# Enigmatisms/AdaPT

Hardware: AMD Instinct MI355X
Metric: Msamples/s (W*H*spp/s), unidirectional MIS path tracing (higher is better)
Workload: dtype f32

## Files before the change

adapt_amd/_lib.py:

```python
from __future__ import annotations

import ctypes as C
import os

_HERE = os.path.dirname(os.path.abspath(__file__))
LIB_PATHS = {"fast": os.environ.get("ADAPT_MI_LIB") or os.path.join(_HERE, "libadapt_mi.so"),
             "exact": os.environ.get("ADAPT_MI_LIB_EXACT") or os.path.join(_HERE, "libadapt_mi_exact.so")}
_variant = "exact" if os.environ.get("APT_EXACT", "0") not in ("", "0") else "fast"
LIB_PATH = LIB_PATHS[_variant]

f32p = C.POINTER(C.c_float)
i32p = C.POINTER(C.c_int32)
u32p = C.POINTER(C.c_uint32)
u8p = C.POINTER(C.c_uint8)
f64p = C.POINTER(C.c_double)
APT_N_KERNELS = 5
KERNEL_NAMES = ("generate", "extend", "shade", "shadow", "finalize")


class AptError(RuntimeError):
    pass


class SceneDesc(C.Structure):
# ... 78 lines not shown
    "apt_device_ptr": (C.c_int, [C.c_void_p, C.POINTER(C.c_void_p), i32p]),
    "apt_stream": (C.c_int, [C.c_void_p, C.POINTER(C.c_void_p)]),
    "apt_intersect": (C.c_int, [C.c_void_p, C.c_int32, f32p, f32p, i32p, f32p, f32p]),
    "apt_occluded": (C.c_int, [C.c_void_p, C.c_int32, f32p, f32p, f32p, i32p]),
    "apt_rng_stream": (C.c_int, [C.c_int32, C.c_uint32, C.c_uint32, C.c_uint32, C.c_int32, u32p]),
    "apt_bxdf_probe": (C.c_int, [C.c_int32, C.c_int32, i32p, f32p, f32p, C.c_float, C.c_int32, C.c_uint32, f32p]),
    "apt_medium_probe": (C.c_int, [C.c_int32, C.c_int32, i32p, f32p, C.c_int32, f32p, C.c_uint32, f32p]),
    "apt_volume_probe": (C.c_int, [C.c_int32, C.c_int32, i32p, f32p, f32p, C.c_int32, f32p, C.c_uint32, f32p]),
    "apt_emitter_probe": (C.c_int, [C.c_void_p, C.c_int32, f32p, C.c_uint32, f32p]),
    "apt_texture_probe": (C.c_int, [C.c_void_p, C.c_int32, i32p, f32p, f32p]),
    "apt_surface_maps_probe": (C.c_int, [C.c_void_p, C.c_int32, i32p, f32p, f32p]),
    "apt_transient_bin_probe": (C.c_int, [C.c_int32, C.c_int32, f32p, C.c_float, C.c_float, C.c_int32, i32p]),
    "apt_renderer_info": (C.c_int, [C.c_void_p, i32p, i32p, C.POINTER(C.c_int64), i32p, C.POINTER(C.c_char_p), i32p]),
    "apt_renderer_camera_fused": (C.c_int, [C.c_void_p, i32p]),
    "apt_renderer_record_staged": (C.c_int, [C.c_void_p, i32p]),
    "apt_measure_sclk_mhz": (C.c_int, [C.c_int32, f32p]),
    "apt_last_error": (C.c_char_p, []),
    "apt_version": (C.c_char_p, []),
}

_libs = {}


def use(variant: str) -> str:
    global _variant, LIB_PATH
    if variant not in LIB_PATHS:
        raise ValueError(f"unknown build variant {variant!r}")
    prev, _variant = _variant, variant
    LIB_PATH = LIB_PATHS[variant]
    return prev
# ... 36 lines not shown
```

adapt_amd/csrc/api.hip:

```cpp
#include <hip/hip_runtime.h>
#include <chrono>

#include <algorithm>
#include <cmath>
#include <cstdio>
#include <cstdlib>
#include <cstring>
#include <limits>
#include <memory>
#include <string>
#include <vector>

#include "../../include/adapt_mi.h"
#include "bvh_build.hpp"
#include "shade_stage.hpp"
#include "unit_kernels.hpp"
#include "aov.hpp"
#include "volumetric.hpp"

#define APT_EXPORT extern "C" __attribute__((visibility("default")))

static thread_local std::string g_err;
static int fail(int code, const std::string& msg) { g_err = msg; return code; }
#define HIP_TRY(expr)                                                                              \
// ... 166 lines not shown
enum Pipeline { PIPE_STAGED, PIPE_SORTED, PIPE_TRACED, PIPE_VOLUMETRIC };

struct apt_renderer {
    const apt_scene* scene = nullptr;
    apt_render_cfg cfg{};
    Params par{};
    int n_cols = 0, npix = 0, spp_batch = 1;
    int cnt = 0;
    std::vector<Lane> lanes;
    int n_lanes = 1;
    hipStream_t stream() const { return lanes[0].stream; }
    DevBuf accum, scratch, pix_key;
    DevBuf cam_strips;
    int record_stage = 0;
    shade_traced_fn traced_fn = nullptr;
    int camera_fuse = 0;
    Counters host_counters{};
    int grid_small = 0, grid_trace = 0, nq = APT_MAX_NQ;
    const ShadeVariant* shade = nullptr;
    int trace_mode = TRACE_BVH;
    int trace_nt = BLOCK;
    int trace_items = BLOCK;
    Pipeline pipeline = PIPE_STAGED;
    int dyn_fetch = 0;
    bool tile_ok = false;
    extend_fn extend = nullptr, fix = nullptr;
    int ovf_levels = 0;
    int n_cq = 0;
    int vev_single = 0;
    vev_shade_fn vev_all = nullptr;
// ... 578 lines not shown
    cf.inv_focal = c.inv_focal; cf.half_w = c.half_w; cf.half_h = c.half_h;
    cf.width = c.width; cf.height = c.height; cf.n_cols = owned_columns(c); cf.band_width = c.band_width; cf.rank = c.rank; cf.world = c.world_size;
    return cf;
}
static int make_camera_strips(apt_renderer* r) {
    if (r->pipeline != PIPE_TRACED) return APT_OK;
    const apt_scene* sc = r->scene;
    const bool cull = !(getenv("APT_CAMERA_CULL") && atoi(getenv("APT_CAMERA_CULL")) == 0);
    std::vector<uint64_t> masks;
    if (apt::camera_strips(sc->h_prims.data(), sc->n_prims, sc->h_flat_recs, sc->h_flat_tab, sc->h_flat_counts, cam_film(r->cfg), cull, masks) != 0)
        return fail(APT_E_INVALID, "apt_renderer_create: camera strip lists: bad record or film");
    hipError_t e = upload(r->cam_strips, masks);
    if (e != hipSuccess) return fail(APT_E_HIP, std::string("upload camera strip lists: ") + hipGetErrorString(e));
    const bool want = !(getenv("APT_CAMERA_FUSE") && atoi(getenv("APT_CAMERA_FUSE")) == 0);
    r->camera_fuse = (want && !r->adaptive && !r->par.do_crop && r->par.max_bounce >= 1 && r->shade->traced_cam != nullptr) ? 1 : 0;
    return APT_OK;
}

APT_EXPORT int apt_camera_strips(const float* prims, int32_t n_prims, const int32_t* obj_info, int32_t n_objects, const apt_render_cfg* cfg, int32_t cull,
                                 uint64_t* masks, int32_t masks_cap, int32_t* n_strips, int32_t* n_pairs) {
    if (!prims || !obj_info || !cfg || n_prims <= 0 || n_objects <= 0 || !n_strips || !n_pairs) return fail(APT_E_INVALID, "apt_camera_strips: bad argument");
    apt_render_cfg c = *cfg;
    if (c.world_size <= 0) { c.world_size = 1; c.rank = 0; }
    if (c.band_width <= 0) c.band_width = c.width;
    if (c.width <= 0 || c.height <= 0 || c.rank < 0 || c.rank >= c.world_size || owned_columns(c) <= 0) return fail(APT_E_INVALID, "apt_camera_strips: bad film or rank");
    std::vector<float> st, tb; int cn[7];
    if (apt::build_flat(prims, n_prims, obj_info, n_objects, nullptr, st, tb, cn) != 0) return fail(APT_E_INVALID, "apt_camera_strips: obj_info range outside the primitive array");
    std::vector<uint64_t> m;
    if (apt::camera_strips(prims, n_prims, st, tb, cn, cam_film(c), cull != 0, m) != 0) return fail(APT_E_INVALID, "apt_camera_strips: bad record or film");
    *n_strips = (int32_t)m.size();
// ... 409 lines not shown
    int done = 0, batch = 0;
    hipEvent_t prev_fin = nullptr;
    const int batch_cap = lane_batch(r, n_spp);
    while (done < n_spp) {
        const int B = (n_spp - done < batch_cap) ? (n_spp - done) : batch_cap;
        Lane& ln = r->lanes[(size_t)(batch % r->n_lanes)];
        hipStream_t st = ln.stream;
        const Queues& q = ln.q;
        Counters* cnt = ln.cnt();
        Params p = r->par; p.cnt_base = r->cnt; p.spp_batch = B;
        const size_t total = (size_t)r->npix * (size_t)B;
        if (int rc = begin_batch(r, ln)) return rc;
#if APT_FAST
        if (r->pipeline == PIPE_TRACED) {
            const unsigned long long* strips = r->cam_strips.as<unsigned long long>();
            int cur = 0, b0 = 0;
            if (r->camera_fuse) {
                { LaunchTimer t(r, APT_K_SHADE, st); hipLaunchKernelGGL(r->shade->traced_cam, dim3(grid_for(total, r->grid_small, nq)), dim3(BLOCK), 0, st, sc, p, q, cnt, strips); }
                { LaunchTimer t(r, APT_K_SHADE, st); hipLaunchKernelGGL(r->traced_fn, dim3(r->grid_fix), dim3(BLOCK), 0, st, sc, p, q, cnt, 0, 0); }
                cur = 1; b0 = 1;
            } else {
                LaunchTimer t(r, APT_K_GENERATE, st);
                if (r->adaptive) hipLaunchKernelGGL(k_generate_trace_ad, dim3(grid_for(total, r->grid_small, 1)), dim3(BLOCK), 0, st, sc, p, q, cnt, (const uint8_t*)r->aq.active, strips);
                else hipLaunchKernelGGL(k_generate_trace, dim3(grid_for(total, r->grid_small, 1)), dim3(BLOCK), 0, st, sc, p, q, cnt, strips);
            }
            for (int b = b0; b < p.max_bounce; b++) {
                { LaunchTimer t(r, APT_K_SHADE, st); hipLaunchKernelGGL(r->traced_fn, dim3(grid_for(total, r->grid_small, nq)), dim3(BLOCK), 0, st, sc, p, q, cnt, cur, b); }
                cur ^= 1;
            }
            if (p.max_bounce > 0) { LaunchTimer t(r, APT_K_SHADOW, st, false); hipLaunchKernelGGL(r->fix, dim3(r->grid_fix), dim3(BLOCK), 0, st, sc, p, q, cnt, cur, (const uint32_t*)cnt->n_active[cur], ln.plan); }
// ... 533 lines not shown
    }
    std::vector<unsigned long long> h((size_t)n_waves * 2);
    HIP_TRY(hipMemcpy(h.data(), out.p, h.size() * 8, hipMemcpyDeviceToHost));
    std::vector<double> r;
    for (int w = 0; w < n_waves; w++) if (h[2 * (size_t)w + 1] > 0) r.push_back(100.0 * (double)h[2 * (size_t)w] / (double)h[2 * (size_t)w + 1]);
    if (r.empty()) return fail(APT_E_STATE, "apt_measure_sclk_mhz: the wall clock did not advance");
    std::nth_element(r.begin(), r.begin() + r.size() / 2, r.end());
    *mhz = (float)r[r.size() / 2];
    return APT_OK;
}
APT_EXPORT int apt_renderer_camera_fused(const apt_renderer* r, int32_t* out) {
    if (!r || !out) return fail(APT_E_INVALID, "apt_renderer_camera_fused: null argument");
    *out = r->camera_fuse;
    return APT_OK;
}
APT_EXPORT int apt_renderer_record_staged(const apt_renderer* r, int32_t* out) {
    if (!r || !out) return fail(APT_E_INVALID, "apt_renderer_record_staged: null argument");
    *out = r->record_stage;
    return APT_OK;
}
APT_EXPORT int apt_renderer_info(const apt_renderer* r, int32_t* spp_batch, int32_t* n_subqueues, int64_t* queue_bytes, int32_t* lds_bytes, const char** shade_variant, int32_t* trace_mode) {
    if (!r) return fail(APT_E_INVALID, "apt_renderer_info: null handle");
    if (spp_batch) *spp_batch = r->spp_batch;
    if (n_subqueues) *n_subqueues = r->nq;
    if (queue_bytes) *queue_bytes = (int64_t)r->lanes[0].pool.bytes * (int64_t)r->lanes.size();
    if (lds_bytes) *lds_bytes = (int32_t)r->lds_bytes;
    if (shade_variant) *shade_variant = r->shade_name.c_str();
    if (trace_mode) *trace_mode = r->trace_mode;
    return APT_OK;
}
// ... 1 lines not shown
```

adapt_amd/csrc/shade_stage.hpp:

```cpp
#pragma once
#include "stages.hpp"

APT_D float ti_fmod(float a, float b) { float q = floorf(a / b); return a - b * q; }
APT_D f3 mix3(f3 a, f3 b, float t) { return a * (1.0f - t) + b * t; }
APT_D f3 texture_query(const DevScene& sc, int map, int obj, float u, float v) {
    const int* ti_ = sc.tex_i + 15 * obj + 5 * map; const float* tf = sc.tex_f + 6 * obj + 2 * map;
    const float w = (float)ti_[3], h = (float)ti_[4];
    const float scaled_u = ti_fmod((u * tf[0]) * w, w - 1.f), scaled_v = ti_fmod((v * tf[1]) * h, h - 1.f);
    float floor_u = floorf(scaled_u), floor_v = floorf(scaled_v);
    const float ratio_u = fmaxf(scaled_u - floor_u, 0.f), ratio_v = fmaxf(scaled_v - floor_v, 0.f);
    floor_u = fminf(fmaxf(floor_u, 0.f), w - 1.f); floor_v = fminf(fmaxf(floor_v, 0.f), h - 1.f);
    const float ceil_u = fminf(floor_u + 1.f, w - 1.f), ceil_v = fminf(floor_v + 1.f, h - 1.f);
    const int fu = (int)(floor_u + (float)ti_[1]), fv = (int)(floor_v + (float)ti_[2]), cu = (int)(ceil_u + (float)ti_[1]), cv = (int)(ceil_v + (float)ti_[2]);
    const float* img = sc.atlas[map]; const int W = sc.atlas_w[map];
    const float* r0 = img + (size_t)fv * W * 3; const float* r1 = img + (size_t)cv * W * 3;
    const f3 q_ff = ld3(r0 + 3 * fu), q_cf = ld3(r0 + 3 * cu), q_fc = ld3(r1 + 3 * fu), q_cc = ld3(r1 + 3 * cu);
    return mix3(mix3(q_ff, q_cf, ratio_u), mix3(q_fc, q_cc, ratio_u), ratio_v);
}
APT_D bool get_uv_item(const DevScene& sc, int map, int obj, int prim, float bu, float bv, f3& out) {
    if (sc.atlas[map] == nullptr || !(sc.tex_i[15 * obj + 5 * map] > -255)) return false;
    const float* uv = sc.uvs + 6 * prim;
    const float w0 = 1.f - bu - bv;
    const float gu = (uv[2] * bu + uv[4] * bv) + uv[0] * w0, gv = (uv[3] * bu + uv[5] * bv) + uv[1] * w0;
    out = texture_query(sc, map, obj, gu, gv);
// ... 50 lines not shown
    if (old >= epoch) {
        while (__hip_atomic_load(&cnt->fix_done[sq * CNT_PAD], __ATOMIC_ACQUIRE, __HIP_MEMORY_SCOPE_AGENT) < epoch) __builtin_amdgcn_s_sleep(16);
        return;
    }
    const uint32_t qbase = (uint32_t)sq * p.subcap, sh_qbase = (uint32_t)sq * q.sh_subcap;
    const bool need_uv = sc.has_vn || sc.tex_i != nullptr;
    for (uint32_t base = 0; base < n_def; base += 64u) {
        const uint32_t li = base + lane_id(); const bool valid = li < n_def;
        const uint32_t lj = valid ? li : n_def - 1u;
        const uint32_t io = (q.tr_stage_top ? qbase + p.subcap - n_def + lj : (uint32_t)ncls * p.cap + qbase + lj) << 4;
        const float4 ra = ldq(q.tr[cur][0], io), rb = ldq(q.tr[cur][1], io), rc = ldq(q.tr[cur][2], io), rd = ldq(q.tr[cur][3], io);
        const f3 o = mk3(ra.x, ra.y, ra.z), d = mk3(rb.x, rb.y, rb.z);
        HitRec r0, r1; r0.t = r1.t = 1e7f; r0.prim = r1.prim = -1; r0.u = r0.v = r1.u = r1.v = 0.f;
        int c0, c1;
        flat_closest2(sc.flat, sc.sweep, sc.prim_class, o, d, o, d, r0, r1, c0, c1);
        if (valid && r0.prim >= 0) {
            const int oc = ncls > 1 ? c0 : 0;
            const uint32_t pos = atomicAdd(&cnt->n_tr[bounce % 3][oc][sq * CNT_PAD], 1u);
            const uint32_t slot = (uint32_t)oc * p.cap + qbase + pos, so = slot << 4;
            stq(q.tr[cur][0], so, make_float4(ra.x, ra.y, ra.z, r0.t));
            stq(q.tr[cur][1], so, make_float4(rb.x, rb.y, rb.z, __uint_as_float((__float_as_uint(rb.w) & ~0xffu) | (uint32_t)r0.prim)));
            stq(q.tr[cur][2], so, rc); stq(q.tr[cur][3], so, rd);
            if (need_uv) { float2 uv_; uv_.x = r0.u; uv_.y = r0.v; stq(q.tr_uv[cur], slot << 3, uv_); }
        } else if (valid && !(rd.x == 0.f && rd.y == 0.f && rd.z == 0.f)) {
            const uint32_t id = __float_as_uint(rc.w), lp_ = id & ((1u << p.pix_bits) - 1u), s_ = id >> p.pix_bits;
            add_radiance(q.L, p.cap, (s_ * (uint32_t)p.npix + lp_) << 2, mk3(rd.x, rd.y, rd.z), true);
        }
    }
    uint32_t t_lit = 0;
    for (uint32_t base = 0; base < n_sh; base += 64u) {
        const uint32_t li = base + lane_id(); const bool valid = li < n_sh;
        const uint32_t io = (sh_qbase + (valid ? li : n_sh - 1u)) << 2;
        const f3 o = ld3q(q.sh_o, q.sh_cap, io), d = ld3q(q.sh_d, q.sh_cap, io), c = ld3q(q.sh_c, q.sh_cap, io);
        const float dist = ldq(q.sh_tmax, io); const uint32_t slot = ldq(q.sh_id, io);
        bool occ, occ_b;
        const float lim = shadow_limit(dist);
        flat_any2(sc.flat, sc.sweep, o, d, o, d, lim, lim, occ, occ_b);
        const bool weird = !(isfinite(c.x) && isfinite(c.y) && isfinite(c.z));
        const bool add = valid && (!occ || weird);
        for (unsigned long long m = __ballot(add); m != 0ull; m &= m - 1ull) {
            if ((int)lane_id() == __ffsll((long long)m) - 1) add_radiance(q.L, p.cap, slot, occ ? c * 0.f : c, true);
        }
        t_lit += (valid && !occ) ? 1u : 0u;
    }
    flush_stat(t_lit, &cnt->stats[sq][ST_LIT]);
    if (lane_id() == 0) __hip_atomic_store(n_sh_p, 0u, __ATOMIC_RELAXED, __HIP_MEMORY_SCOPE_AGENT);
    __threadfence();
    if (lane_id() == 0) __hip_atomic_store(&cnt->fix_done[sq * CNT_PAD], epoch, __ATOMIC_RELEASE, __HIP_MEMORY_SCOPE_AGENT);
}
#endif
struct ShadeArgs3 { DevScene sc; Params p; Queues q; };
typedef const __attribute__((address_space(4))) ShadeArgs3* args3_ptr;
APT_D args3_ptr kernel_args3() { return (args3_ptr)__builtin_amdgcn_kernarg_segment_ptr(); }
APT_D const ShadeArgs3* args_fresh(args3_ptr a) {
    asm volatile("" : "+s"(a));
    return (const ShadeArgs3*)a;
// ... 170 lines not shown
    }
#ifdef APT_ROWTOP_STATS
    t_loop0 = __builtin_amdgcn_s_memtime();
#endif
    for (uint32_t base = sl.first; base < n; base += sl.stride) {
        APT_ARGS_PHASE();
        const uint32_t pos = base + threadIdx.x, idx = qbase + pos;
        bool alive = pos < n;
        const uint32_t cu_pm = pf_pm;
        float4 cu_ra = make_float4(0.f, 0.f, 0.f, 0.f), cu_rb = cu_ra;
        if (PFP) { const int rp = max(tr_prim(cu_pm), 0); cu_ra = (A_->sc).prim_shade[2 * rp]; cu_rb = (A_->sc).prim_shade[2 * rp + 1]; prefetch_prim(base + sl.stride); }
        Vertex vx; vertex_reset(vx);
        Rng rng; rng_init(rng, 0u, 0u, 0u, 0u);
        f3 Lc = splat3(0.f);
        bool entry = alive;
        float ray_pdf = 1.f;
        if constexpr (CAM) {
            const uint32_t w = (uint32_t)__builtin_amdgcn_readfirstlane((int)(pos >> 6)) * (uint32_t)(A_->p).nq + (uint32_t)sl.q;
            const uint32_t id_ = w * 64u + lane_id();
            const bool valid = alive && id_ < cam_total;
            f3 dir = mk3(0.f, 0.f, 1.f);
            uint32_t draws = 0;
            uint32_t jitter_tail[2] = {0u, 0u};
            if (valid) {
                const uint32_t lp = id_ % (uint32_t)(A_->p).npix, s = id_ / (uint32_t)(A_->p).npix;
                int i, j; local_to_global((A_->p), lp, i, j);
                for (int pl = 0; pl < (A_->p).l_planes; pl++) stL((A_->q).L, (A_->p).cap, (id_ << 2) | (uint32_t)pl, splat3(0.f));
                dir = camera_ray_dir((A_->p), i, j, s, draws, WINDOW ? jitter_tail : nullptr);
                vx.id = (s << (A_->p).pix_bits) | lp;
            }
            if (draws) atomicAdd(&s_draws[threadIdx.x >> 6], draws);
            const f3 cam_o = mk3((A_->p).cam_t[0], (A_->p).cam_t[1], (A_->p).cam_t[2]);
            float c_t = 0.f; int c_run = -1, c_idx = -1;
            if (__any(valid)) c_idx = flat_closest1<true>((A_->sc).flat, cam_o, dir, 1e7f, c_t, c_run, camera_strip_mask((A_->p), strips, w));
            const bool c_defer = valid && (c_run >= 0 || flat_needs_cull((A_->sc).flat, dir));
            HitRec hr; hr.t = 1e7f; hr.prim = -1; hr.u = hr.v = 0.f;
            int hit_cls = 0;
            if (valid && !c_defer && c_idx >= 0) flat_resolve((A_->sc).flat, c_idx, c_t, cam_o, dir, hr, hit_cls);
            { const uint32_t nv = wave_count(valid); t_samples += nv; t_extend += nv; }
            if (__any(c_defer)) {
                const int ncls = (A_->q).tr_ncls;
                const uint32_t dpos = wave_append(c_defer, &cnt->n_tr[0][ncls][sl.q * CNT_PAD]);
                if (c_defer) {
                    const uint32_t slot = (A_->q).tr_stage_top ? qbase + (A_->p).subcap - 1u - dpos : (uint32_t)ncls * (A_->p).cap + qbase + dpos, so = slot << 4;
                    stq((A_->q).tr[0][0], so, make_float4(cam_o.x, cam_o.y, cam_o.z, hr.t));
                    stq((A_->q).tr[0][1], so, make_float4(dir.x, dir.y, dir.z, __uint_as_float(tr_pack(hr.prim, draws, false))));
                    stq((A_->q).tr[0][2], so, make_float4(1.f, 1.f, 1.f, __uint_as_float(vx.id)));
                    float one = 1.f;
                    if (WINDOW) asm volatile("" : "+v"(one));
                    stq((A_->q).tr[0][3], so, make_float4(0.f, 0.f, 0.f, one));
                    if ((A_->sc).has_vn || (A_->sc).tex_i != nullptr) { float2 uv_; uv_.x = hr.u; uv_.y = hr.v; stq((A_->q).tr_uv[0], slot << 3, uv_); }
                }
            }
            entry = valid && !c_defer;
            alive = entry && hr.prim >= 0;
            if (alive) {
                vx.o = cam_o; vx.d = dir; vx.thr = splat3(1.f);
                f3 rec_kd; float2 uv; uv.x = hr.u; uv.y = hr.v;
                build_hit((A_->sc), hr.prim, hr.t, uv.x, uv.y, vx.o, vx.d, vx.it, vx.hit_light, rec_kd);
                alive = open_vertex<BM, SM, TEX>(A_, vx, rng, hr.prim, rec_kd, tr_meta(tr_pack(hr.prim, draws, false), 0u), ray_pdf, uv, 0, WINDOW ? jitter_tail : nullptr);
            }
// ... 2 lines not shown
        if constexpr (STAGE) {
            staged_read(s_rec + lane_id(), sa, sb, sc_, sd);
            { const int rp = max(tr_prim(__float_as_uint(sb.w)), 0); rec4 pa, pb; staged_read2(s_prim + 2 * rp, pa, pb); cu_ra = make_float4(pa.x, pa.y, pa.z, pa.w); cu_rb = make_float4(pb.x, pb.y, pb.z, pb.w); }
            if (alive && bounce > 0) { Lc = mk3(sd.x, sd.y, sd.z); if (SM & APT_SRC_AREA) ray_pdf = sd.w; }
        }
        if (!CAM && !STAGE && alive && bounce > 0) { const float4 dd = ldq(trD, idx << 4); Lc = mk3(dd.x, dd.y, dd.z); if (SM & APT_SRC_AREA) ray_pdf = dd.w; }
        if (!CAM && alive) {
            float4 a, b_, c;
            if constexpr (STAGE) { a = make_float4(sa.x, sa.y, sa.z, sa.w); b_ = make_float4(sb.x, sb.y, sb.z, sb.w); c = make_float4(sc_.x, sc_.y, sc_.z, sc_.w); }
            else { a = ldq(trA, idx << 4); b_ = ldq(trB, idx << 4); c = ldq(trC, idx << 4); }
#ifdef APT_ROWTOP_STATS
            if constexpr (!STAGE) { const unsigned long long t0_ = __builtin_amdgcn_s_memtime(); staged_wait(); t_rowtop += __builtin_amdgcn_s_memtime() - t0_; t_rows++; }
#endif
            vx.o = mk3(a.x, a.y, a.z); vx.d = mk3(b_.x, b_.y, b_.z); vx.thr = mk3(c.x, c.y, c.z); vx.id = __float_as_uint(c.w);
            const uint32_t pm = PFP ? cu_pm : __float_as_uint(b_.w);
            const int prim = tr_prim(pm);
            if (prim < 0) alive = false;
            else {
                f3 rec_kd; float2 uv; uv.x = uv.y = 0.f;
                if ((A_->sc).has_vn || (TEX && (A_->sc).tex_i != nullptr)) uv = ldq((A_->q).tr_uv[cur], idx << 3);
                if (PFP || STAGE) build_hit_rec((A_->sc), cu_ra, cu_rb, prim, a.w, uv.x, uv.y, vx.o, vx.d, vx.it, vx.hit_light, rec_kd);
                else build_hit((A_->sc), prim, a.w, uv.x, uv.y, vx.o, vx.d, vx.it, vx.hit_light, rec_kd);
                alive = open_vertex<BM, SM, TEX>(A_, vx, rng, prim, rec_kd, tr_meta(pm, (uint32_t)bounce), ray_pdf, uv, bounce);
            }
        }
        tl.shade += wave_count(alive);
#ifdef APT_NEAR_STATS
        t_near += wave_count(alive && bounce > 0 && vx.it.min_depth < 2e-3f);
#endif
        if (alive) vx.hit_point = vx.d * vx.it.min_depth + vx.o;
// ... 38 lines not shown
            cont = cont && (tr_idx >= 0 || tr_defer);
            if (cont && !tr_defer) { HitRec hr; flat_resolve((A_->sc).flat, tr_idx, tr_t, vx.hit_point, new_d, hr, hit_cls); tr_hit = hr.prim; tr_u = hr.u; tr_v = hr.v; }
            tr_q = !cont ? -1 : (tr_defer ? 1 : 0);
            { const Append a_ = append_issue(tr_q == 0, next_counter); tr_app.raw = a_.raw; tr_app.rank = rank_in(a_.m); }
        }
        APT_ARGS_PHASE();
        {
            const bool defer = f.want && flat_needs_cull((A_->sc).flat, f.dir);
            bool occ = false;
            if (__any(f.want && !defer)) {
                const FlatList ls = (occ_e >= 0) ? flat_occ_list((A_->sc).flat, occ_e) : flat_full_list((A_->sc).flat);
                occ = flat_any1(ls, vx.hit_point, f.dir, shadow_limit(f.dist));
            }
            if (__any(defer)) {
                const uint32_t spos = wave_append(defer, &cnt->n_fix_sh[cur][sl.q * CNT_PAD]);
                if (defer && spos < (A_->q).sh_subcap) { const uint32_t so = (sh_qbase + spos) << 2; shadow_store((A_->q), so, vx.hit_point, f.dir, f.dist, f.contrib); stq((A_->q).sh_id, so, vx.l_off); }
            }
            const bool traced = f.want && !defer;
            if (traced) {
                const bool weird = !(isfinite(f.contrib.x) && isfinite(f.contrib.y) && isfinite(f.contrib.z));
                if (!occ || weird) Lc = Lc + (occ ? f.contrib * 0.f : f.contrib);
            }
            t_traced += wave_count(f.want); t_lit += wave_count(traced && !occ);
        }
        if constexpr (STAGE) {
#ifdef APT_ROWTOP_STATS
            const unsigned long long t0_ = __builtin_amdgcn_s_memtime();
#endif
            staged_wait();
#ifdef APT_ROWTOP_STATS
            t_rowtop += __builtin_amdgcn_s_memtime() - t0_; t_rows++;
#endif
        }
        uint32_t npos = (uint32_t)__builtin_amdgcn_readlane((int)tr_app.raw, 0) + tr_app.rank;
        if (__any(tr_q == 1)) { const uint32_t dpos = wave_append(tr_q == 1, next_counter + APT_MAX_NQ * CNT_PAD); if (tr_q == 1) npos = dpos; }
        if (cont) {
            const uint32_t slot = (tr_q == 1) ? qbase + (A_->p).subcap - 1u - npos : qbase + npos, so = slot << 4;
            stq((A_->q).tr[nxt][0], so, make_float4(vx.hit_point.x, vx.hit_point.y, vx.hit_point.z, tr_t));
            stq((A_->q).tr[nxt][1], so, make_float4(new_d.x, new_d.y, new_d.z, __uint_as_float(tr_pack(tr_hit, rng.draw, is_spec))));
            stq((A_->q).tr[nxt][2], so, make_float4(vx.thr.x, vx.thr.y, vx.thr.z, __uint_as_float(vx.id)));
            stq((A_->q).tr[nxt][3], so, make_float4(Lc.x, Lc.y, Lc.z, new_pdf));
            if ((A_->sc).has_vn || (A_->sc).tex_i != nullptr) { float2 uv_; uv_.x = tr_u; uv_.y = tr_v; stq((A_->q).tr_uv[nxt], slot << 3, uv_); }
        }
        if (!cont && entry && !(Lc.x == 0.f && Lc.y == 0.f && Lc.z == 0.f)) {
            const uint32_t lp_ = vx.id & ((1u << (A_->p).pix_bits) - 1u), s_ = vx.id >> (A_->p).pix_bits;
            add_radiance((A_->q).L, (A_->p).cap, (s_ * (uint32_t)(A_->p).npix + lp_) << 2, Lc, true);
        }
    }
    flush_uniform(t_traced, &cnt->stats[sl.q][ST_SHADOW_TRACED]); flush_uniform(t_lit, &cnt->stats[sl.q][ST_LIT]);
    flush_uniform(t_extend, &cnt->stats[sl.q][ST_EXTEND]);
    if (CAM) flush_uniform(t_samples, &cnt->stats[sl.q][ST_SAMPLES]);
    tally_flush(tl, s_draws, cnt, sl.q);
#ifdef APT_NEAR_STATS
    flush_uniform(t_near, &cnt->stats[sl.q][14]);
#endif
#ifdef APT_ROWTOP_STATS
    if (!CAM && lane_id() == 0 && t_rows) {
        atomicAdd(&cnt->stats[sl.q][12], t_rowtop); atomicAdd(&cnt->stats[sl.q][13], (unsigned long long)__builtin_amdgcn_s_memtime() - t_loop0); atomicAdd(&cnt->stats[sl.q][14], t_rows);
    }
#endif
}
// ... 181 lines not shown
```

adapt_amd/csrc/stages.hpp:

```cpp
#pragma once
#include <hip/hip_runtime.h>

#include "rng.hpp"
#include "shading.hpp"
#include "traverse.hpp"
#include "vec.hpp"

struct DevMedium {
    int type;
    float ior;
    f3 u_s, u_a, u_e, par, pdf;
};
struct DevVolume {
    int type, xres, yres, zres;
    f3 albedo, trans, mini, maxi, majorant, pdf;
    f3 inv_r0, inv_r1, inv_r2;
    DevMedium ph;
    const float* grid;
};
struct DevScene {
    DevBvh bvh;
    SweepScene sweep;
    FlatScene flat;
    const float* normals;
// ... 29 lines not shown
    float rr_threshold;
    uint32_t seed;
    int cnt_base, spp_batch;
    uint32_t cap;
    uint32_t subcap;
    int nq;
    uint32_t pix_bits;
    const uint32_t* pix_key;
    float inv_ns, inv_ns1;
    int fix_par;
    int volumetric_flat;
    int nee_vm;
    int l_planes;
    int traced;
    float w_min[3], w_max[3];
};

struct Queues {
    float* ray_o[2]; float* ray_d[2];
    float* hit_t; int* hit_prim; float* hit_u; float* hit_v;
    float4* tr[2][4]; float2* tr_uv[2]; int tr_ncls, tr_stage_top;
    uint32_t* fix_ext; uint32_t* fix_sh;
    float* thr[2]; uint32_t* id[2]; uint32_t* meta[2]; float* pdf[2];
    float* sh_o; float* sh_d; float* sh_tmax; float* sh_c; uint32_t* sh_id;
    uint32_t* sh_walk[2];
    float* L;
    uint32_t sh_cap, sh_subcap;
    float4* cq[4];
    int n_classes;
};
#define APT_MAX_CLASSES 8
// ... 33 lines not shown
    uint32_t fix_claim[APT_MAX_NQ * CNT_PAD];
    uint32_t fix_done[APT_MAX_NQ * CNT_PAD];
    unsigned long long stats[APT_MAX_NQ][16];
#ifdef APT_WALK_STATS
    unsigned long long wdbg[2][8];
#endif
};

APT_D uint32_t pack_meta(uint32_t draw, uint32_t bounce, bool spec) { return (draw & 0xffffu) | ((bounce & 0xffu) << 16) | (spec ? (1u << 24) : 0u); }

#define BLOCK 256
#define TR_NO_PRIM 0xffu
APT_D uint32_t tr_pack(int prim, uint32_t draw, bool spec) { return (prim < 0 ? TR_NO_PRIM : (uint32_t)prim) | ((draw & 0xffffu) << 8) | (spec ? (1u << 24) : 0u); }
APT_D int tr_prim(uint32_t pm) { return ((pm & 0xffu) == TR_NO_PRIM) ? -1 : (int)(pm & 0xffu); }
APT_D uint32_t tr_meta(uint32_t pm, uint32_t bounce) { return pack_meta(pm >> 8, bounce, ((pm >> 24) & 1u) != 0u); }
#ifndef APT_EXCLUSIVE_L
#define APT_EXCLUSIVE_L(p) ((p).S == 1 || (p).l_planes == (p).S)
#endif

struct LdsPlan { int stack_depth; uint2* ovf; int ovf_stride; };
extern __shared__ float4 s_dyn[];
typedef __attribute__((address_space(3))) float lds_f;
APT_D TravStack make_stack(const LdsPlan& plan) {
    TravStack ts;
    ts.lds = (lds_u2*)(reinterpret_cast<grp_t*>(s_dyn)) + threadIdx.x;
    ts.stride = BLOCK; ts.k = plan.stack_depth; ts.ovf_stride = plan.ovf_stride;
    ts.ovf = plan.ovf ? (glb_u2*)(reinterpret_cast<grp_t*>(plan.ovf) + (blockIdx.x * blockDim.x + threadIdx.x)) : (glb_u2*)nullptr;
    ts.lut = (lds_u8*)nullptr;
    return ts;
}
// ... 1 lines not shown
    TravStack ts = make_stack(plan);
    ts.lut = (lds_u8*)(reinterpret_cast<float*>(s_dyn) + (size_t)plan.stack_depth * BLOCK * 2 + 6 * BLOCK);
    fill_permute_lut(ts.lut);
    __syncthreads();
    return ts;
}

APT_D uint32_t lane_id() { return threadIdx.x & 63u; }
APT_D float* L_slot(float* L, uint32_t cap, uint32_t code) { return L + (size_t)(code & 3u) * 4 * cap + (size_t)(code & ~3u); }
APT_D f3 ldL(float* L, uint32_t cap, uint32_t code) { const float4 v = *reinterpret_cast<const float4*>(L_slot(L, cap, code)); return mk3(v.x, v.y, v.z); }
APT_D void stL(float* L, uint32_t cap, uint32_t code, f3 v) { *reinterpret_cast<float4*>(L_slot(L, cap, code)) = make_float4(v.x, v.y, v.z, 0.f); }
APT_D void add_radiance(float* L, uint32_t cap, uint32_t code, f3 c, bool exclusive) {
    if (exclusive) { const f3 a = ldL(L, cap, code); stL(L, cap, code, mk3(a.x + c.x, a.y + c.y, a.z + c.z)); }
    else { float* p_ = L_slot(L, cap, code); atomicAdd(p_, c.x); atomicAdd(p_ + 1, c.y); atomicAdd(p_ + 2, c.z); }
}
APT_D float shadow_limit(float dist) { return (dist > 0.0f) ? dist - 1e-4f : 1e7f; }
APT_D bool non_finite(f3 c) { return !(isfinite(c.x) && isfinite(c.y) && isfinite(c.z)); }
APT_D uint32_t rank_in(unsigned long long m) { return __builtin_amdgcn_mbcnt_hi((uint32_t)(m >> 32), __builtin_amdgcn_mbcnt_lo((uint32_t)m, 0u)); }
APT_D uint32_t wave_append(bool flag, uint32_t* counter) {
    unsigned long long m = __ballot(flag);
    uint32_t base = 0;
    if (lane_id() == 0 && m) base = atomicAdd(counter, (uint32_t)__popcll(m));
    base = (uint32_t)__builtin_amdgcn_readlane((int)base, 0);
    return base + rank_in(m);
}

struct Append { unsigned long long m; uint32_t raw; };
APT_D Append append_issue(bool flag, uint32_t* counter) {
    Append a; a.m = __ballot(flag); a.raw = 0;
    if (lane_id() == 0 && a.m) a.raw = atomicAdd(counter, (uint32_t)__popcll(a.m));
// ... 205 lines not shown
            if (__any(alive)) {
                const unsigned long long mask = camera_strip_mask(p, strips, w);
                tr_idx = flat_closest1<true>(sc->flat, cam_o, dir, 1e7f, tr_t, tr_run, mask);
            }
            const bool defer = alive && (tr_run >= 0 || flat_needs_cull(sc->flat, dir));
            HitRec hr; hr.t = 1e7f; hr.prim = -1; hr.u = hr.v = 0.f;
            int hit_cls = 0;
            if (alive && !defer && tr_idx >= 0) flat_resolve(sc->flat, tr_idx, tr_t, cam_o, dir, hr, hit_cls);
            const int ocls = !alive ? -1 : (defer ? q.tr_ncls : (hr.prim >= 0 ? (q.tr_ncls > 1 ? hit_cls : 0) : -1));
            const TrAppend app = tr_append_issue(ocls, q.tr_ncls + 1, &cnt->n_tr[0][0][sq * CNT_PAD], APT_MAX_NQ * CNT_PAD);
            pos = tr_append_pos(app, ocls);
            if (alive) t_samples++;
            if (ocls >= 0) {
                const uint32_t slot = (q.tr_stage_top && ocls == q.tr_ncls) ? (uint32_t)sq * p.subcap + p.subcap - 1u - pos : (uint32_t)ocls * p.cap + (uint32_t)sq * p.subcap + pos, so = slot << 4;
                stq(q.tr[0][0], so, make_float4(cam_o.x, cam_o.y, cam_o.z, hr.t));
                stq(q.tr[0][1], so, make_float4(dir.x, dir.y, dir.z, __uint_as_float(tr_pack(hr.prim, draws, false))));
                stq(q.tr[0][2], so, make_float4(1.f, 1.f, 1.f, __uint_as_float(((idx / (uint32_t)p.npix) << p.pix_bits) | (idx % (uint32_t)p.npix))));
                stq(q.tr[0][3], so, make_float4(0.f, 0.f, 0.f, 1.f));
                if (sc->has_vn || sc->tex_i != nullptr) { float2 uv_; uv_.x = hr.u; uv_.y = hr.v; stq(q.tr_uv[0], slot << 3, uv_); }
            }
        }
#endif
        if (alive && !TRACE) {
            const uint32_t so = ((uint32_t)sq * p.subcap + pos) << 2;
            st3q(q.ray_o[0], p.cap, so, mk3(p.cam_t[0], p.cam_t[1], p.cam_t[2]));
            st3q(q.ray_d[0], p.cap, so, dir);
            st3q(q.thr[0], p.cap, so, splat3(1.f));
            stq(q.id[0], so, ((idx / (uint32_t)p.npix) << p.pix_bits) | (idx % (uint32_t)p.npix));
            stq(q.meta[0], so, pack_meta(draws, 0u, false));
            stq(q.pdf[0], so, 1.f);
            t_samples++;
// ... 559 lines not shown
```

adapt_amd/renderer.py:

```python
from __future__ import annotations

import ctypes as C
import time
from typing import List, Optional

import numpy as np

from . import _lib
from .scene_pack import FlatScene, RenderConfig, make_config, pack_scene
from .tiles import TilePlan

__all__ = ["Renderer", "VolumeRenderer", "DeviceScene", "bxdf_probe", "medium_probe", "volume_probe", "rng_stream", "adaptive_config", "adaptive_segments", "relative_error", "DENOISE_DEFAULTS"]

ADAPTIVE_DEFAULTS = {"min_spp": 64, "step": 32}
DENOISE_DEFAULTS = {"firefly_threshold": 0.0, "iterations": 3, "sigma_n": 128.0, "sigma_z": 0.1, "sigma_a": 0.1, "sigma_c": 1.0, "demodulate": True}
TRAVERSAL_NAMES = dict(enumerate(("bvh", "sweep", "tile", "flat")))


def adaptive_config(adaptive) -> Optional[dict]:
    if adaptive is None or adaptive is False:
        return None
    if not isinstance(adaptive, dict):
        raise TypeError("adaptive must be None or a dict {'threshold': t, 'min_spp': 64, 'step': 32}")
    unknown = set(adaptive) - {"threshold", "min_spp", "step"}
# ... 458 lines not shown
        return {"spp_per_batch": b.value, "n_subqueues": nq.value, "queue_bytes": qb.value, "lds_bytes": lds.value,
                "shade_variant": name.value.decode() if name.value else "",
                "traversal": TRAVERSAL_NAMES.get(tm.value, str(tm.value)), "arithmetic": self.arithmetic,
                "sampling": "adaptive" if self.adaptive else "uniform", **({"adaptive": dict(self.adaptive)} if self.adaptive else {})}

    def camera_fused(self) -> bool:
        f = C.c_int32(0)
        _lib.check(self.lib.apt_renderer_camera_fused(self.handle, C.byref(f)), "apt_renderer_camera_fused", self.lib)
        return bool(f.value)

    def record_staged(self) -> bool:
        f = C.c_int32(0)
        _lib.check(self.lib.apt_renderer_record_staged(self.handle, C.byref(f)), "apt_renderer_record_staged", self.lib)
        return bool(f.value)

    def get_check_point(self) -> dict:
        return {"w": self.w, "h": self.h, "crop_x": self.crop_x, "crop_y": self.crop_y, "crop_rx": self.crop_rx,
                "crop_ry": self.crop_ry, "focal": self.focal, "num_objects": self.num_objects, "num_prims": self.num_prims,
                "cam_orient": np.array(self.cam_orient), "src_num": self.src_num, "cam_t": np.array(self.cam_t),
                "accumulation": self.color.to_numpy(), "counter": self._cnt,
                **({"transient_bins": self.tile_transient()} if self.n_bins else {}),
                **({"aov_sums": self.tile_aov(), "aov_samples": self._aov_n} if self._aov_n else {}),
                **(self._adaptive_check_point() if self.adaptive else {})}

    _ADAPTIVE_KEYS = ("adaptive", "sample_counts", "moments", "active")

    def _adaptive_check_point(self) -> dict:
        n, act = self.tile_sample_counts(with_mask=True)
        return {"adaptive": dict(self.adaptive), "sample_counts": n, "moments": self.tile_moments(), "active": act}

# ... 53 lines not shown
```

include/adapt_mi.h:

```cpp
#ifndef ADAPT_MI_H
#define ADAPT_MI_H

#include <stdint.h>

#ifdef __cplusplus
extern "C" {
#endif

#define APT_OK            0
#define APT_E_INVALID    -1
#define APT_E_NO_DEVICE  -2
#define APT_E_HIP        -3
#define APT_E_NOMEM      -4
#define APT_E_STATE      -5

typedef struct apt_bvh apt_bvh;
typedef struct apt_scene apt_scene;
typedef struct apt_renderer apt_renderer;

typedef struct apt_scene_desc {
    int32_t n_prims, n_objects, n_sources, has_vertex_normal;
    const float*   prims;
    const float*   normals;
    const float*   v_normals;
// ... 122 lines not shown
int apt_rng_stream(int32_t device, uint32_t pixel, uint32_t seed, uint32_t sample, int32_t n, uint32_t* out);
int apt_bxdf_probe(int32_t device, int32_t n, const int32_t* bxdf_i, const float* bxdf_f, const float* dirs12,
                   float world_ior, int32_t do_sample, uint32_t seed, float* out);
int apt_texture_probe(const apt_scene*, int32_t n, const int32_t* map_obj, const float* uv, float* out3);
int apt_surface_maps_probe(const apt_scene*, int32_t n, const int32_t* prim_first, const float* bary, float* out7);
int apt_medium_probe(int32_t device, int32_t n, const int32_t* med_i, const float* med_f, int32_t mode, const float* in7,
                     uint32_t seed, float* out8);
int apt_volume_probe(int32_t device, int32_t n, const int32_t* vol_i, const float* vol_f, const float* vol_grid, int32_t mode,
                     const float* in10, uint32_t seed, float* out8);
int apt_emitter_probe(const apt_scene*, int32_t n, const float* in11, uint32_t seed, float* out12);
int apt_transient_bin_probe(int32_t device, int32_t n, const float* t, float min_time, float interval, int32_t n_bins, int32_t* out);
int apt_renderer_info(const apt_renderer*, int32_t* spp_batch, int32_t* n_subqueues, int64_t* queue_bytes,
                      int32_t* lds_bytes, const char** shade_variant, int32_t* trace_mode);
int apt_renderer_camera_fused(const apt_renderer*, int32_t* fused);
int apt_renderer_record_staged(const apt_renderer*, int32_t* staged);

int apt_measure_sclk_mhz(int32_t device, float* mhz);

const char* apt_last_error(void);
const char* apt_version(void);

#ifdef __cplusplus
}
#endif
#endif
```

Baseline: 6108.

## Defer radiance buffer zeroing to first write via a written flag

Camera-fused shading no longer zeroes every pixel's L slot up front. Each path carries a TR_WRITTEN bit, and the first contribution (miss, terminal radiance, or a shadow result tagged SH_STORE) stores directly instead of accumulating. This removes the per-sample zeroing stores and the read-modify-write on first deposit. The cost is extra flag plumbing through the ray and shadow queues, and correctness now relies on every path writing its slot exactly once first, so a debug env option fills L with a NaN sentinel to catch missed writes.

```diff
diff --git a/adapt_amd/_lib.py b/adapt_amd/_lib.py
--- a/adapt_amd/_lib.py
+++ b/adapt_amd/_lib.py
@@ -116,6 +116,7 @@
     "apt_renderer_info": (C.c_int, [C.c_void_p, i32p, i32p, C.POINTER(C.c_int64), i32p, C.POINTER(C.c_char_p), i32p]),
     "apt_renderer_camera_fused": (C.c_int, [C.c_void_p, i32p]),
     "apt_renderer_record_staged": (C.c_int, [C.c_void_p, i32p]),
+    "apt_renderer_radiance_store": (C.c_int, [C.c_void_p, i32p]),
     "apt_measure_sclk_mhz": (C.c_int, [C.c_int32, f32p]),
     "apt_last_error": (C.c_char_p, []),
     "apt_version": (C.c_char_p, []),
diff --git a/adapt_amd/csrc/api.hip b/adapt_amd/csrc/api.hip
--- a/adapt_amd/csrc/api.hip
+++ b/adapt_amd/csrc/api.hip
@@ -204,6 +204,8 @@
     DevBuf cam_strips;
     int record_stage = 0;
     shade_traced_fn traced_fn = nullptr;
+    int radiance_store = 0;
+    int l_sentinel = 0;
     int camera_fuse = 0;
     Counters host_counters{};
     int grid_small = 0, grid_trace = 0, nq = APT_MAX_NQ;
@@ -812,6 +814,10 @@
     if (e != hipSuccess) return fail(APT_E_HIP, std::string("upload camera strip lists: ") + hipGetErrorString(e));
     const bool want = !(getenv("APT_CAMERA_FUSE") && atoi(getenv("APT_CAMERA_FUSE")) == 0);
     r->camera_fuse = (want && !r->adaptive && !r->par.do_crop && r->par.max_bounce >= 1 && r->shade->traced_cam != nullptr) ? 1 : 0;
+    const bool want_store = !(getenv("APT_RADIANCE_STORE") && atoi(getenv("APT_RADIANCE_STORE")) == 0);
+    r->radiance_store = (want_store && r->camera_fuse) ? 1 : 0;
+    r->par.radiance_store = r->radiance_store;
+    r->l_sentinel = (getenv("APT_L_SENTINEL") && atoi(getenv("APT_L_SENTINEL")) != 0) ? 1 : 0;
     return APT_OK;
 }
 
@@ -1251,6 +1257,7 @@
 #if APT_FAST
         if (r->pipeline == PIPE_TRACED) {
             const unsigned long long* strips = r->cam_strips.as<unsigned long long>();
+            if (r->l_sentinel) { unchain(r, st); HIP_TRY(hipMemsetAsync(q.L, 0xFF, (size_t)p.cap * 16 * (size_t)p.l_planes, st)); }
             int cur = 0, b0 = 0;
             if (r->camera_fuse) {
                 { LaunchTimer t(r, APT_K_SHADE, st); hipLaunchKernelGGL(r->shade->traced_cam, dim3(grid_for(total, r->grid_small, nq)), dim3(BLOCK), 0, st, sc, p, q, cnt, strips); }
@@ -1814,6 +1821,11 @@
     *out = r->camera_fuse;
     return APT_OK;
 }
+APT_EXPORT int apt_renderer_radiance_store(const apt_renderer* r, int32_t* out) {
+    if (!r || !out) return fail(APT_E_INVALID, "apt_renderer_radiance_store: null argument");
+    *out = r->radiance_store;
+    return APT_OK;
+}
 APT_EXPORT int apt_renderer_record_staged(const apt_renderer* r, int32_t* out) {
     if (!r || !out) return fail(APT_E_INVALID, "apt_renderer_record_staged: null argument");
     *out = r->record_stage;
diff --git a/adapt_amd/csrc/shade_stage.hpp b/adapt_amd/csrc/shade_stage.hpp
--- a/adapt_amd/csrc/shade_stage.hpp
+++ b/adapt_amd/csrc/shade_stage.hpp
@@ -88,17 +88,20 @@
         HitRec r0, r1; r0.t = r1.t = 1e7f; r0.prim = r1.prim = -1; r0.u = r0.v = r1.u = r1.v = 0.f;
         int c0, c1;
         flat_closest2(sc.flat, sc.sweep, sc.prim_class, o, d, o, d, r0, r1, c0, c1);
+        const bool written = (__float_as_uint(rb.w) & TR_WRITTEN) != 0u;
+        const uint32_t id = __float_as_uint(rc.w), l_off = ((id >> p.pix_bits) * (uint32_t)p.npix + (id & ((1u << p.pix_bits) - 1u))) << 2;
         if (valid && r0.prim >= 0) {
             const int oc = ncls > 1 ? c0 : 0;
+            if (!written) stL(q.L, p.cap, l_off, splat3(0.f));
             const uint32_t pos = atomicAdd(&cnt->n_tr[bounce % 3][oc][sq * CNT_PAD], 1u);
             const uint32_t slot = (uint32_t)oc * p.cap + qbase + pos, so = slot << 4;
             stq(q.tr[cur][0], so, make_float4(ra.x, ra.y, ra.z, r0.t));
-            stq(q.tr[cur][1], so, make_float4(rb.x, rb.y, rb.z, __uint_as_float((__float_as_uint(rb.w) & ~0xffu) | (uint32_t)r0.prim)));
+            stq(q.tr[cur][1], so, make_float4(rb.x, rb.y, rb.z, __uint_as_float((__float_as_uint(rb.w) & ~0xffu) | TR_WRITTEN | (uint32_t)r0.prim)));
             stq(q.tr[cur][2], so, rc); stq(q.tr[cur][3], so, rd);
             if (need_uv) { float2 uv_; uv_.x = r0.u; uv_.y = r0.v; stq(q.tr_uv[cur], slot << 3, uv_); }
-        } else if (valid && !(rd.x == 0.f && rd.y == 0.f && rd.z == 0.f)) {
-            const uint32_t id = __float_as_uint(rc.w), lp_ = id & ((1u << p.pix_bits) - 1u), s_ = id >> p.pix_bits;
-            add_radiance(q.L, p.cap, (s_ * (uint32_t)p.npix + lp_) << 2, mk3(rd.x, rd.y, rd.z), true);
+        } else if (valid) {
+            if (!written) stL(q.L, p.cap, l_off, mk3(rd.x, rd.y, rd.z));
+            else if (!(rd.x == 0.f && rd.y == 0.f && rd.z == 0.f)) add_radiance(q.L, p.cap, l_off, mk3(rd.x, rd.y, rd.z), true);
         }
     }
     uint32_t t_lit = 0;
@@ -106,14 +109,18 @@
         const uint32_t li = base + lane_id(); const bool valid = li < n_sh;
         const uint32_t io = (sh_qbase + (valid ? li : n_sh - 1u)) << 2;
         const f3 o = ld3q(q.sh_o, q.sh_cap, io), d = ld3q(q.sh_d, q.sh_cap, io), c = ld3q(q.sh_c, q.sh_cap, io);
-        const float dist = ldq(q.sh_tmax, io); const uint32_t slot = ldq(q.sh_id, io);
+        const float dist = ldq(q.sh_tmax, io); const uint32_t code = ldq(q.sh_id, io), slot = code & ~3u;
+        const bool store = (code & SH_STORE) != 0u;
         bool occ, occ_b;
         const float lim = shadow_limit(dist);
         flat_any2(sc.flat, sc.sweep, o, d, o, d, lim, lim, occ, occ_b);
         const bool weird = !(isfinite(c.x) && isfinite(c.y) && isfinite(c.z));
         const bool add = valid && (!occ || weird);
-        for (unsigned long long m = __ballot(add); m != 0ull; m &= m - 1ull) {
-            if ((int)lane_id() == __ffsll((long long)m) - 1) add_radiance(q.L, p.cap, slot, occ ? c * 0.f : c, true);
+        for (unsigned long long m = __ballot(add || (valid && store)); m != 0ull; m &= m - 1ull) {
+            if ((int)lane_id() == __ffsll((long long)m) - 1) {
+                if (store) store_radiance(q.L, p.cap, slot, add ? (occ ? c * 0.f : c) : splat3(0.f));
+                else add_radiance(q.L, p.cap, slot, occ ? c * 0.f : c, true);
+            }
         }
         t_lit += (valid && !occ) ? 1u : 0u;
     }
@@ -314,6 +321,7 @@
         Rng rng; rng_init(rng, 0u, 0u, 0u, 0u);
         f3 Lc = splat3(0.f);
         bool entry = alive;
+        bool written = CAM ? (A_->p).radiance_store == 0 : false;
         float ray_pdf = 1.f;
         if constexpr (CAM) {
             const uint32_t w = (uint32_t)__builtin_amdgcn_readfirstlane((int)(pos >> 6)) * (uint32_t)(A_->p).nq + (uint32_t)sl.q;
@@ -325,7 +333,7 @@
             if (valid) {
                 const uint32_t lp = id_ % (uint32_t)(A_->p).npix, s = id_ / (uint32_t)(A_->p).npix;
                 int i, j; local_to_global((A_->p), lp, i, j);
-                for (int pl = 0; pl < (A_->p).l_planes; pl++) stL((A_->q).L, (A_->p).cap, (id_ << 2) | (uint32_t)pl, splat3(0.f));
+                if (written) for (int pl = 0; pl < (A_->p).l_planes; pl++) stL((A_->q).L, (A_->p).cap, (id_ << 2) | (uint32_t)pl, splat3(0.f));
                 dir = camera_ray_dir((A_->p), i, j, s, draws, WINDOW ? jitter_tail : nullptr);
                 vx.id = (s << (A_->p).pix_bits) | lp;
             }
@@ -344,7 +352,7 @@
                 if (c_defer) {
                     const uint32_t slot = (A_->q).tr_stage_top ? qbase + (A_->p).subcap - 1u - dpos : (uint32_t)ncls * (A_->p).cap + qbase + dpos, so = slot << 4;
                     stq((A_->q).tr[0][0], so, make_float4(cam_o.x, cam_o.y, cam_o.z, hr.t));
-                    stq((A_->q).tr[0][1], so, make_float4(dir.x, dir.y, dir.z, __uint_as_float(tr_pack(hr.prim, draws, false))));
+                    stq((A_->q).tr[0][1], so, make_float4(dir.x, dir.y, dir.z, __uint_as_float(tr_pack(hr.prim, draws, false) | (written ? TR_WRITTEN : 0u))));
                     stq((A_->q).tr[0][2], so, make_float4(1.f, 1.f, 1.f, __uint_as_float(vx.id)));
                     float one = 1.f;
                     if (WINDOW) asm volatile("" : "+v"(one));
@@ -377,6 +385,7 @@
 #endif
             vx.o = mk3(a.x, a.y, a.z); vx.d = mk3(b_.x, b_.y, b_.z); vx.thr = mk3(c.x, c.y, c.z); vx.id = __float_as_uint(c.w);
             const uint32_t pm = PFP ? cu_pm : __float_as_uint(b_.w);
+            written = (pm & TR_WRITTEN) != 0u;
             const int prim = tr_prim(pm);
             if (prim < 0) alive = false;
             else {
@@ -445,7 +454,9 @@
             }
             if (__any(defer)) {
                 const uint32_t spos = wave_append(defer, &cnt->n_fix_sh[cur][sl.q * CNT_PAD]);
-                if (defer && spos < (A_->q).sh_subcap) { const uint32_t so = (sh_qbase + spos) << 2; shadow_store((A_->q), so, vx.hit_point, f.dir, f.dist, f.contrib); stq((A_->q).sh_id, so, vx.l_off); }
+                const bool listed = defer && spos < (A_->q).sh_subcap, first = listed && tr_q == 0 && !written;
+                if (listed) { const uint32_t so = (sh_qbase + spos) << 2; shadow_store((A_->q), so, vx.hit_point, f.dir, f.dist, f.contrib); stq((A_->q).sh_id, so, vx.l_off | (first ? SH_STORE : 0u)); }
+                written = written || first;
             }
             const bool traced = f.want && !defer;
             if (traced) {
@@ -468,14 +479,15 @@
         if (cont) {
             const uint32_t slot = (tr_q == 1) ? qbase + (A_->p).subcap - 1u - npos : qbase + npos, so = slot << 4;
             stq((A_->q).tr[nxt][0], so, make_float4(vx.hit_point.x, vx.hit_point.y, vx.hit_point.z, tr_t));
-            stq((A_->q).tr[nxt][1], so, make_float4(new_d.x, new_d.y, new_d.z, __uint_as_float(tr_pack(tr_hit, rng.draw, is_spec))));
+            stq((A_->q).tr[nxt][1], so, make_float4(new_d.x, new_d.y, new_d.z, __uint_as_float(tr_pack(tr_hit, rng.draw, is_spec) | (written ? TR_WRITTEN : 0u))));
             stq((A_->q).tr[nxt][2], so, make_float4(vx.thr.x, vx.thr.y, vx.thr.z, __uint_as_float(vx.id)));
             stq((A_->q).tr[nxt][3], so, make_float4(Lc.x, Lc.y, Lc.z, new_pdf));
             if ((A_->sc).has_vn || (A_->sc).tex_i != nullptr) { float2 uv_; uv_.x = tr_u; uv_.y = tr_v; stq((A_->q).tr_uv[nxt], slot << 3, uv_); }
         }
-        if (!cont && entry && !(Lc.x == 0.f && Lc.y == 0.f && Lc.z == 0.f)) {
+        if (!cont && entry && !(written && Lc.x == 0.f && Lc.y == 0.f && Lc.z == 0.f)) {
             const uint32_t lp_ = vx.id & ((1u << (A_->p).pix_bits) - 1u), s_ = vx.id >> (A_->p).pix_bits;
-            add_radiance((A_->q).L, (A_->p).cap, (s_ * (uint32_t)(A_->p).npix + lp_) << 2, Lc, true);
+            if (!written) stL((A_->q).L, (A_->p).cap, (s_ * (uint32_t)(A_->p).npix + lp_) << 2, Lc);
+            else add_radiance((A_->q).L, (A_->p).cap, (s_ * (uint32_t)(A_->p).npix + lp_) << 2, Lc, true);
         }
     }
     flush_uniform(t_traced, &cnt->stats[sl.q][ST_SHADOW_TRACED]); flush_uniform(t_lit, &cnt->stats[sl.q][ST_LIT]);
diff --git a/adapt_amd/csrc/stages.hpp b/adapt_amd/csrc/stages.hpp
--- a/adapt_amd/csrc/stages.hpp
+++ b/adapt_amd/csrc/stages.hpp
@@ -67,7 +67,9 @@
     int l_planes;
     int traced;
     float w_min[3], w_max[3];
+    int radiance_store;
 };
+static_assert(sizeof(Params) == 240, "Params::radiance_store fills the tail padding: the kernels' argument offsets behind Params stay where they were");
 
 struct Queues {
     float* ray_o[2]; float* ray_d[2];
@@ -131,6 +133,8 @@
 APT_D uint32_t tr_pack(int prim, uint32_t draw, bool spec) { return (prim < 0 ? TR_NO_PRIM : (uint32_t)prim) | ((draw & 0xffffu) << 8) | (spec ? (1u << 24) : 0u); }
 APT_D int tr_prim(uint32_t pm) { return ((pm & 0xffu) == TR_NO_PRIM) ? -1 : (int)(pm & 0xffu); }
 APT_D uint32_t tr_meta(uint32_t pm, uint32_t bounce) { return pack_meta(pm >> 8, bounce, ((pm >> 24) & 1u) != 0u); }
+#define TR_WRITTEN (1u << 25)
+#define SH_STORE 1u
 #ifndef APT_EXCLUSIVE_L
 #define APT_EXCLUSIVE_L(p) ((p).S == 1 || (p).l_planes == (p).S)
 #endif
@@ -162,6 +166,7 @@
     if (exclusive) { const f3 a = ldL(L, cap, code); stL(L, cap, code, mk3(a.x + c.x, a.y + c.y, a.z + c.z)); }
     else { float* p_ = L_slot(L, cap, code); atomicAdd(p_, c.x); atomicAdd(p_ + 1, c.y); atomicAdd(p_ + 2, c.z); }
 }
+APT_D void store_radiance(float* L, uint32_t cap, uint32_t code, f3 v) { stL(L, cap, code, mk3(0.f + v.x, 0.f + v.y, 0.f + v.z)); }
 APT_D float shadow_limit(float dist) { return (dist > 0.0f) ? dist - 1e-4f : 1e7f; }
 APT_D bool non_finite(f3 c) { return !(isfinite(c.x) && isfinite(c.y) && isfinite(c.z)); }
 APT_D uint32_t rank_in(unsigned long long m) { return __builtin_amdgcn_mbcnt_hi((uint32_t)(m >> 32), __builtin_amdgcn_mbcnt_lo((uint32_t)m, 0u)); }
@@ -397,7 +402,7 @@
             if (ocls >= 0) {
                 const uint32_t slot = (q.tr_stage_top && ocls == q.tr_ncls) ? (uint32_t)sq * p.subcap + p.subcap - 1u - pos : (uint32_t)ocls * p.cap + (uint32_t)sq * p.subcap + pos, so = slot << 4;
                 stq(q.tr[0][0], so, make_float4(cam_o.x, cam_o.y, cam_o.z, hr.t));
-                stq(q.tr[0][1], so, make_float4(dir.x, dir.y, dir.z, __uint_as_float(tr_pack(hr.prim, draws, false))));
+                stq(q.tr[0][1], so, make_float4(dir.x, dir.y, dir.z, __uint_as_float(tr_pack(hr.prim, draws, false) | TR_WRITTEN)));
                 stq(q.tr[0][2], so, make_float4(1.f, 1.f, 1.f, __uint_as_float(((idx / (uint32_t)p.npix) << p.pix_bits) | (idx % (uint32_t)p.npix))));
                 stq(q.tr[0][3], so, make_float4(0.f, 0.f, 0.f, 1.f));
                 if (sc->has_vn || sc->tex_i != nullptr) { float2 uv_; uv_.x = hr.u; uv_.y = hr.v; stq(q.tr_uv[0], slot << 3, uv_); }
diff --git a/adapt_amd/renderer.py b/adapt_amd/renderer.py
--- a/adapt_amd/renderer.py
+++ b/adapt_amd/renderer.py
@@ -496,6 +496,11 @@
         _lib.check(self.lib.apt_renderer_record_staged(self.handle, C.byref(f)), "apt_renderer_record_staged", self.lib)
         return bool(f.value)
 
+    def radiance_store(self) -> bool:
+        f = C.c_int32(0)
+        _lib.check(self.lib.apt_renderer_radiance_store(self.handle, C.byref(f)), "apt_renderer_radiance_store", self.lib)
+        return bool(f.value)
+
     def get_check_point(self) -> dict:
         return {"w": self.w, "h": self.h, "crop_x": self.crop_x, "crop_y": self.crop_y, "crop_rx": self.crop_rx,
                 "crop_ry": self.crop_ry, "focal": self.focal, "num_objects": self.num_objects, "num_prims": self.num_prims,
diff --git a/include/adapt_mi.h b/include/adapt_mi.h
--- a/include/adapt_mi.h
+++ b/include/adapt_mi.h
@@ -160,6 +160,7 @@
                       int32_t* lds_bytes, const char** shade_variant, int32_t* trace_mode);
 int apt_renderer_camera_fused(const apt_renderer*, int32_t* fused);
 int apt_renderer_record_staged(const apt_renderer*, int32_t* staged);
+int apt_renderer_radiance_store(const apt_renderer*, int32_t* store);
 
 int apt_measure_sclk_mhz(int32_t device, float* mhz);
 
```

Result: no change. 6155 (median of 6 runs) (+0.8%).
